# MathisWellmann/gym-rs

Measured on AMD Instinct MI355X. Metric: env-steps/sec (whole node), CartPole-v1 @ 2^20 envs per MI355X, higher is better.
Workload: dtype f32

## Files before the change

### gym-rs_amd/csrc/gymrs_engine.hip

```cpp
#include "gymrs_engine_priv.h"

static thread_local std::string g_last_error;

gymrs_status fail(gymrs_status st, const std::string& msg)
{
    g_last_error = msg;
    return st;
}


constexpr int kMaxDevices = 64;
static std::atomic<const gymrs_engine*> g_last_stepper[kMaxDevices];
static std::atomic<uint32_t> g_stepper_run[kMaxDevices];
constexpr uint32_t kTakeOverAfter = 64;

static size_t action_size(gymrs_env_kind kind) { return kind == GYMRS_PENDULUM ? sizeof(float) : sizeof(uint8_t); }

constexpr uint64_t kHostPoolMaxLanes = 64;

static uint64_t os_entropy()
{
    std::random_device rd;
    return ((uint64_t)rd() << 32) ^ (uint64_t)rd();
}
// ... 75 lines not shown
}

gymrs_status fold_reset_log(gymrs_engine* e)
{
    if (!e->reset_log || e->log_pending == 0) return GYMRS_OK;
    if (gymrs_status st = stream_op_barrier(e)) return st;
    HIP_TRY(launch_fold_reset_log(e->reset_log, e->log_row_words, e->log_first_tick, e->log_pending, e->log_vec, e->ep_start, e->n,
                                  e->block_stats, e->stream));
    e->log_pending = 0;
    return GYMRS_OK;
}

static bool launch_is_logged(const gymrs_engine* e, uint32_t flags)
{
    return e->reset_log && (flags & GYMRS_TRACK_STATS) && (flags & GYMRS_AUTO_RESET) && !(flags & GYMRS_TIME_LIMIT);
}

static gymrs_status log_before_step(gymrs_engine* e, uint32_t flags, uint32_t* fold)
{
    *fold = 0;
    if (!e->reset_log) return GYMRS_OK;
    const ResetLogStep s = reset_log_step({e->log_pending, e->log_first_tick, e->log_vec}, launch_is_logged(e, flags), e->tick, e->vec);
    if (s.fold_first)
        if (gymrs_status st = fold_reset_log(e)) return st;
    e->log_pending = s.after.pending;
    e->log_first_tick = s.after.first_tick;
    e->log_vec = s.after.vec;
    *fold = s.fold_step;
    return GYMRS_OK;
}
// ... 458 lines not shown
    }
    e->n_stat_blocks = (uint32_t)((((n_envs + 255) / 256) + 15) / 16 * 16);
    chk(dev_alloc(&e->block_stats, (size_t)e->n_stat_blocks * 2));
    constexpr uint32_t kAllThree = GYMRS_AUTO_RESET | GYMRS_TRACK_STATS | GYMRS_TIME_LIMIT;
    e->limit_elidable = kind == GYMRS_CARTPOLE && (flags & kAllThree) == kAllThree;
    {
        constexpr uint64_t kElideRewardFromBytes = 128ull << 20;
        bool on = kind == GYMRS_CARTPOLE && (flags & GYMRS_AUTO_RESET) && bytes_per_step(kind, e->state_dim, n_envs) >= kElideRewardFromBytes;
        if (const char* v = std::getenv("GYMRS_DEV_ELIDE_REWARD"))
            if (kind == GYMRS_CARTPOLE && (flags & GYMRS_AUTO_RESET) && (v[0] == '0' || v[0] == '1')) on = v[0] == '1';
        e->elide_reward = on;
    }
    if ((flags & GYMRS_TRACK_STATS) && (flags & GYMRS_AUTO_RESET) && kind == GYMRS_CARTPOLE &&
        (!(flags & GYMRS_TIME_LIMIT) || e->limit_elidable)) {
        e->log_row_words = e->n_stat_blocks * 4;
        chk(dev_alloc(&e->reset_log, (size_t)kResetLogRows * e->log_row_words));
    }
    if (e->limit_elidable) {
        chk(dev_alloc(&e->age_dev, (size_t)kStatsPartials));
        if (st == GYMRS_OK && mapped_host_block(2 * sizeof(uint32_t), &e->age_host, &e->age_host_dev) != hipSuccess)
            st = fail(GYMRS_EHIP, "hipHostMalloc (age words)");
    }
    chk(dev_alloc(&e->wave_open, (size_t)e->n_stat_blocks));
    chk(dev_alloc(&e->wave_clean, (size_t)e->n_stat_blocks));
    chk(dev_alloc(&e->err, 2));
    if (st == GYMRS_OK && mapped_host_block(2 * sizeof(uint32_t), &e->err_seen, &e->err_seen_dev) != hipSuccess)
        st = fail(GYMRS_EHIP, "hipHostMalloc (error flags)");
    chk(dev_alloc(&e->stats_dev, 4));
    if (st == GYMRS_OK && mapped_host_block(4 * sizeof(double), &e->stats_host, &e->stats_host_dev) != hipSuccess)
        st = fail(GYMRS_EHIP, "hipHostMalloc (statistics read-out)");
    chk(dev_alloc(&e->stats_acc, (size_t)kStatsPartials * 3));
    chk(dev_alloc(&e->stats_base, (size_t)kStatsBaseWords));
    chk(dev_alloc(&e->tick_dev, 1));
    if (st != GYMRS_OK) {
        std::string msg = g_last_error;
        gymrs_engine_destroy(e);
        return fail(st, msg);
    }
    hipError_t serr = hipStreamCreateWithFlags(&e->stream, hipStreamNonBlocking);
    if (serr != hipSuccess) {
        gymrs_engine_destroy(e);
        return fail(GYMRS_EHIP, std::string("hipStreamCreate: ") + hipGetErrorString(serr));
    }
    e->own_stream = true;
    static const uint32_t err_init[2] = {0u, 0xffffffffu};
    hipError_t merr = hipMemcpyAsync(e->err, err_init, sizeof(err_init), hipMemcpyHostToDevice, e->stream);
    if (merr == hipSuccess && e->reset_log) merr = hipMemsetAsync(e->reset_log, 0, (size_t)kResetLogRows * e->log_row_words * 8, e->stream);
    if (merr == hipSuccess) merr = hipMemsetAsync(e->truncated, 0, npad, e->stream);
    if (merr == hipSuccess) merr = hipMemsetAsync(e->stats_dev, 0, 4 * sizeof(double), e->stream);
    if (merr != hipSuccess) {
        gymrs_engine_destroy(e);
        return fail(GYMRS_EHIP, std::string("engine init: ") + hipGetErrorString(merr));
    }
    st = gymrs_reset(e, 0, 0, nullptr, nullptr);
    if (st == GYMRS_OK) st = gymrs_sync(e);
    if (st != GYMRS_OK) {
        std::string msg = g_last_error;
        gymrs_engine_destroy(e);
        return fail(st, msg);
    }
    if (aql_enabled_by_env() && !e->pool_host) {
        e->aql_tried = true;
// ... 23 lines not shown
gymrs_status gymrs_get_stream(gymrs_engine* e, void** hip_stream)
{
    if (!e || !hip_stream) return fail(GYMRS_EINVAL, "gymrs_get_stream: NULL argument");
    *hip_stream = e->stream;
    return GYMRS_OK;
}

gymrs_status gymrs_set_tuning(gymrs_engine* e, int lanes_per_thread, int memory_hint)
{
    if (!e) return fail(GYMRS_EINVAL, "gymrs_set_tuning: engine is NULL");
    if (lanes_per_thread != 4 && lanes_per_thread != 8)
        return fail(GYMRS_EINVAL, "gymrs_set_tuning: lanes_per_thread must be 4 or 8");
    if (memory_hint < 0 || memory_hint > 3) return fail(GYMRS_EINVAL, "gymrs_set_tuning: memory_hint must be 0, 1, 2 or 3");
    e->vec = lanes_per_thread;
    e->nt_mode = memory_hint;
    return GYMRS_OK;
}

static double default_reset_low_f64(gymrs_env_kind kind, int) { return kind == GYMRS_CARTPOLE ? -0.05 : -0.6; }
static double default_reset_high_f64(gymrs_env_kind kind, int) { return kind == GYMRS_CARTPOLE ? 0.05 : -0.4; }

struct PcgReset {
    const uint64_t* seeds_dev;
    double low[4], scale[4];
};

static gymrs_status reset_lanes(gymrs_engine* e, uint64_t seed, const float* lo, const float* hi, const PcgReset* pcg)
{
    std::memcpy(e->lo, lo, sizeof(e->lo));
    std::memcpy(e->hi, hi, sizeof(e->hi));
    if (gymrs_status st = fold_reset_log(e)) return st;
    e->seed = seed;
    e->tick = 0;
    if (e->graph_exec) {
        (void)hipGraphExecDestroy(e->graph_exec);
        e->graph_exec = nullptr;
    }

    ResetArgs a;
    std::memset(&a, 0, sizeof(a));
    for (int j = 0; j < 4; ++j) a.s[j] = e->s[j];
    a.obs_cos = e->obs_cos;
    a.obs_sin = e->obs_sin;
    a.reward = e->reward;
    a.done = e->done;
    a.truncated = e->truncated;
    a.beyond = e->beyond;
    a.ep_start = e->ep_start;
// ... 115 lines not shown
    e->open_vec = vec;
    return GYMRS_OK;
}

struct StepLaunch {
    uint32_t flags;
    StepArgs args;
};

static gymrs_status prepare_step(gymrs_engine* e, const void* actions, bool chain, StepLaunch* l)
{
    l->flags = take_over_device(e, launch_flags_of(e));
    if (gymrs_status st = elide_time_limit(e, &l->flags)) return st;
    if (chain) l->flags = (l->flags & ~kFlagHintMask) | hint_bits(e->nt_mode, bytes_per_step(e->kind, e->state_dim, e->n), true);
    l->args = step_args(e, actions);
    return log_before_step(e, l->flags, &l->args.fold_step);
}

static void record_step(gymrs_engine* e, const StepLaunch& l, int path)
{
    e->last_flags = l.flags;
    e->last_path = path;
    if (has_uniform_clock(e)) {
        e->trunc_held = (int)l.args.truncate_all;
        e->uniform_start = uniform_clock_after(e->tick, e->uniform_start, l.args.truncate_all != 0, (e->flags & GYMRS_AUTO_RESET) != 0);
    }
    e->tick += 1;
    if (path == 2) e->aql_launches += 1;
    e->n_steps_total += (double)e->n;
}

static hipError_t launch_step_through_hip_module(gymrs_engine* e, uint32_t flags, const StepArgs& a);

static gymrs_status step_through_hip(gymrs_engine* e, const void* actions)
{
    StepLaunch l;
    if (gymrs_status st = prepare_step(e, actions, false, &l)) return st;
    const uint32_t flags = l.flags;
    const StepArgs& a = l.args;
    if ((e->dev_hooks & 8u) && !(e->flags & GYMRS_FINAL_OBS) && !e->table_k)
        HIP_TRY(launch_step_through_hip_module(e, flags, a));
    else
// ... 34 lines not shown
    Policy,
    Exploring,
};
struct RolloutRequest {
    ActionSource actions;
    uint64_t action_seed = 0, action_t0 = 0;
    bool fitness = false;
    const gymrs_trajectory* record = nullptr;
    const TransitionArgs* transitions = nullptr;
};

static gymrs_status rollout_impl(gymrs_engine* e, uint32_t n_steps, const RolloutRequest& q)
{
    if (n_steps == 0) return GYMRS_OK;
    HIP_TRY(hipSetDevice(e->device));
    StepArgs a = step_args(e, nullptr);
    a.skip_trunc_store = 0;
    RolloutArgs r;
    std::memset(&r, 0, sizeof(r));
    r.action_seed = q.action_seed;
    r.action_t0 = q.action_t0;
    r.uniform_start = e->uniform_start;
    r.n_steps = n_steps;
    r.n_actions = e->kind == GYMRS_CARTPOLE ? 2u : 3u;
    r.max_torque = e->max_torque;
    int vec = e->vec == 8 ? 8 : 4;
    if (const gymrs_trajectory* rec = q.record) {
        r.rec_obs = rec->obs;
        r.rec_action = rec->actions;
        r.rec_reward = rec->reward;
// ... 147 lines not shown
    HIP_TRY(hipMemcpyAsync(e->action_staging, actions_host, bytes, hipMemcpyHostToDevice, e->stream));
    return gymrs_step(e, e->action_staging);
}

static gymrs_status build_graph(gymrs_engine* e, const char* base, uint64_t stride_bytes, uint32_t n_buffers, uint32_t steps)
{
    if (e->graph_exec) {
        (void)hipGraphExecDestroy(e->graph_exec);
        e->graph_exec = nullptr;
    }
    hipGraph_t graph = nullptr;
    HIP_TRY(hipStreamBeginCapture(e->stream, hipStreamCaptureModeThreadLocal));
    hipError_t err = hipSuccess;
    const uint32_t flags = launch_flags_of(e);
    ResetLogRing ring{0, 0, e->vec};
    for (uint32_t t = 0; t < steps && err == hipSuccess; ++t) {
        StepArgs a = step_args(e, base + (size_t)(t % n_buffers) * stride_bytes);
        a.tick = t;
        a.tick_base = e->tick_dev;
        const ResetLogStep s = reset_log_step(ring, launch_is_logged(e, flags), t, e->vec);
        a.fold_step = s.fold_step;
        ring = s.after;
        err = launch_step(e->kind, e->vec, flags, a, launch_consts(e), e->stream);
    }
    if (err == hipSuccess) err = launch_tick_advance(e->tick_dev, steps, e->stream);
    hipError_t end = hipStreamEndCapture(e->stream, &graph);
    if (err != hipSuccess || end != hipSuccess) {
        if (graph) (void)hipGraphDestroy(graph);
        return fail(GYMRS_EHIP, std::string("HIP graph capture: ") + hipGetErrorString(err != hipSuccess ? err : end));
    }
    err = hipGraphInstantiate(&e->graph_exec, graph, nullptr, nullptr, 0);
    (void)hipGraphDestroy(graph);
    if (err != hipSuccess) return fail(GYMRS_EHIP, std::string("hipGraphInstantiate: ") + hipGetErrorString(err));
    e->graph_actions = base;
    e->graph_stride = stride_bytes;
    e->graph_nbuf = n_buffers;
    e->graph_steps = steps;
// ... 163 lines not shown
        if (n_steps >= per_graph) {
            const bool hit = e->graph_exec && e->graph_actions == base && e->graph_stride == stride_bytes &&
                             e->graph_nbuf == n_buffers && e->graph_steps == per_graph && e->graph_flags == launch_flags_of(e) &&
                             e->graph_vec == e->vec && e->graph_seed == e->seed;
            if (!hit) {
                if (gymrs_status st = build_graph(e, base, stride_bytes, n_buffers, per_graph)) return st;
            }
            const unsigned long long tick_now = e->tick;
            HIP_TRY(hipMemcpyAsync(e->tick_dev, &tick_now, sizeof(tick_now), hipMemcpyHostToDevice, e->stream));
            HIP_TRY(hipStreamSynchronize(e->stream));
            if (gymrs_status st = fold_reset_log(e)) return st;
            if (e->device >= 0 && e->device < kMaxDevices) {
                g_last_stepper[e->device].store(e, std::memory_order_relaxed);
                g_stepper_run[e->device].store(kTakeOverAfter, std::memory_order_relaxed);
            }
            while (n_steps - done >= per_graph) {
                HIP_TRY(hipGraphLaunch(e->graph_exec, e->stream));
                done += per_graph;
                e->tick += per_graph;
                e->n_steps_total += (double)e->n * (double)per_graph;
            }
            if (e->flags & GYMRS_TIME_LIMIT) e->trunc_zero = false;
        }
    }
    if (!use_graph && aql_usable(e, n_steps - done)) {
        bool taken = false;
        if (gymrs_status st = step_many_aql(e, base, stride_bytes, n_buffers, done, n_steps, &taken)) return st;
        if (taken) done = n_steps;
    }
    for (uint32_t t = done; t < n_steps; ++t)
// ... 60 lines not shown
```

### gym-rs_amd/csrc/gymrs_engine_io.hip

```cpp
#include "gymrs_engine_priv.h"
#include "gymrs_evaluate.h"

static RcclApi g_rccl;

void comm_destroy(gymrs_engine* e)
{
    if (e->comm && g_rccl.CommDestroy) g_rccl.CommDestroy(e->comm);
    e->comm = nullptr;
}

extern "C" {

gymrs_status gymrs_obs_ptrs(gymrs_engine* e, float** out_ptrs, int* obs_dim)
{
    if (!e || !out_ptrs || !obs_dim) return fail(GYMRS_EINVAL, "gymrs_obs_ptrs: NULL argument");
    if (e->kind == GYMRS_PENDULUM) {
        out_ptrs[0] = e->obs_cos;
        out_ptrs[1] = e->obs_sin;
        out_ptrs[2] = e->s[1];
    } else {
        for (int j = 0; j < e->obs_dim; ++j) out_ptrs[j] = e->s[j];
    }
    *obs_dim = e->obs_dim;
    return GYMRS_OK;
// ... 90 lines not shown
        if (gymrs_status st_ = stream_sync_checked(e)) return st_;
        for (int j = 0; j < e->state_dim; ++j) std::memcpy(host_out + (size_t)j * count, host_of(e, e->s[j]) + first, count * sizeof(float));
        return GYMRS_OK;
    }
    for (int j = 0; j < e->state_dim; ++j)
        HIP_TRY(hipMemcpyAsync(host_out + (size_t)j * count, e->s[j] + first, count * sizeof(float), hipMemcpyDeviceToHost, e->stream));
    if (gymrs_status st_ = stream_sync_checked(e)) return st_;
    return GYMRS_OK;
}

gymrs_status gymrs_set_state(gymrs_engine* e, uint64_t first, uint64_t count, const float* host_in)
{
    if (!e || !host_in) return fail(GYMRS_EINVAL, "gymrs_set_state: NULL argument");
    if (gymrs_status st = range_check(e, first, count, "gymrs_set_state")) return st;
    HIP_TRY(hipSetDevice(e->device));
    if (e->pool_host) {
        HIP_TRY(hipStreamSynchronize(e->stream));
        for (int j = 0; j < e->state_dim; ++j) std::memcpy(host_of(e, e->s[j]) + first, host_in + (size_t)j * count, count * sizeof(float));
        if (e->kind == GYMRS_PENDULUM)
            for (uint64_t i = 0; i < count; ++i) sincosf_(host_in[i], host_of(e, e->obs_sin) + first + i, host_of(e, e->obs_cos) + first + i);
        return GYMRS_OK;
    }
    for (int j = 0; j < e->state_dim; ++j)
        HIP_TRY(hipMemcpyAsync(e->s[j] + first, host_in + (size_t)j * count, count * sizeof(float), hipMemcpyHostToDevice, e->stream));
    if (e->kind == GYMRS_PENDULUM) {
        std::vector<float> c(count), s(count);
        for (uint64_t i = 0; i < count; ++i) sincosf_(host_in[i], &s[i], &c[i]);
        HIP_TRY(hipMemcpyAsync(e->obs_cos + first, c.data(), count * sizeof(float), hipMemcpyHostToDevice, e->stream));
        HIP_TRY(hipMemcpyAsync(e->obs_sin + first, s.data(), count * sizeof(float), hipMemcpyHostToDevice, e->stream));
        HIP_TRY(hipStreamSynchronize(e->stream));
// ... 88 lines not shown
    dst->max_steps = src->max_steps;
    std::memcpy(dst->lo, src->lo, sizeof(dst->lo));
    std::memcpy(dst->hi, src->hi, sizeof(dst->hi));
    std::memcpy(dst->dflt_lo, src->dflt_lo, sizeof(dst->dflt_lo));
    std::memcpy(dst->dflt_hi, src->dflt_hi, sizeof(dst->dflt_hi));
    dst->epoch = src->epoch;
    dst->seed = src->seed;
    dst->tick = src->tick;
    dst->uniform_start = src->uniform_start;
    dst->n_steps_total = src->n_steps_total;
    dst->vec = src->vec;
    dst->nt_mode = src->nt_mode;
    dst->open_vec = src->open_vec;
    dst->trunc_held = src->trunc_held;
    limit_restart(dst, src->start_bound, src->trunc_zero);
    *dst->err_seen = 1u;
}
}
}

gymrs_status gymrs_engine_clone(gymrs_engine* src, gymrs_engine** out)
{
    if (!src || !out) return fail(GYMRS_EINVAL, "gymrs_engine_clone: NULL argument");
    *out = nullptr;
    gymrs_engine* dst = nullptr;
    if (gymrs_status st = gymrs_engine_create(src->kind, src->n, src->gid0, src->device, nullptr, src->flags, &dst)) return st;
    copy_scalars(dst, src);
    if (gymrs_status st = fold_reset_log(src)) {
        gymrs_engine_destroy(dst);
        return st;
// ... 117 lines not shown
    if (table_k) {
        p += sizeof(table_k);
        if (gymrs_status st = gymrs_set_param_table(e, p, (uint32_t)table_k)) return st;
        p += (size_t)table_k * params_size(e->kind);
        HIP_TRY(hipMemcpyAsync(e->param_index, p, (size_t)e->n * sizeof(uint16_t), hipMemcpyHostToDevice, e->stream));
    } else {
        if (e->table_k) drop_graph(e);
        e->table_k = 0;
    }
    HIP_TRY(hipStreamSynchronize(e->stream));
    e->gid0 = h.gid0;
    e->epoch = h.epoch;
    e->max_steps = h.max_steps;
    e->seed = h.seed;
    e->tick = h.tick;
    e->uniform_start = h.uniform_start;
    e->n_steps_total = h.n_steps_total;
    std::memcpy(e->lo, h.lo, sizeof(e->lo));
    std::memcpy(e->hi, h.hi, sizeof(e->hi));
    e->max_torque = h.max_torque;
    e->open_vec = (int)h.open_vec;
    e->trunc_held = -1;
    limit_restart(e, 0, false);
    *e->err_seen = 1u;
    HIP_TRY(hipMemsetAsync(e->wave_clean, 0, (size_t)e->n_stat_blocks * sizeof(uint32_t), e->stream));
    e->clean_shape = 0;
    std::memcpy(&e->consts, h.consts, h.consts_bytes);
    std::memcpy(&e->params, h.params, sizeof(e->params));
    return GYMRS_OK;
}
// ... 455 lines not shown
                                        "time and keeps a lane's step count in 32 bits); split the evaluation");
    if (gymrs_status st = ensure_policy_eval(e, "gymrs_evaluate_policy")) return st;
    HIP_TRY(hipSetDevice(e->device));
    HIP_TRY(launch_policy_eval_identity(e->eval_dev, e->policy.n_policies, e->stream));
    EvalArgs a;
    std::memset(&a, 0, sizeof(a));
    a.n = e->n;
    a.gid0 = e->gid0;
    a.seed = d->seed;
    a.episodes = d->episodes_per_lane;
    a.max_steps = m;
    a.flags = d->flags & GYMRS_EVAL_COMMON_STARTS;
    a.lengths = d->lengths_dev;
    a.table = e->eval_dev;
    a.box = make_sample_box(e->dflt_lo, e->dflt_hi, e->state_dim);
    HIP_TRY(launch_evaluate_policy(e->kind, e->table_k ? kFlagTable : 0u, a, launch_consts(e), e->policy, e->stream));
    return GYMRS_OK;
}

gymrs_status gymrs_policy_eval_ptr(gymrs_engine* e, gymrs_policy_eval** dev_out, uint32_t* n_policies)
{
    if (!e || !dev_out) return fail(GYMRS_EINVAL, "gymrs_policy_eval_ptr: NULL argument");
    if (gymrs_status st = ensure_policy_eval(e, "gymrs_policy_eval_ptr")) return st;
    *dev_out = e->eval_dev;
    if (n_policies) *n_policies = e->policy.n_policies;
    return GYMRS_OK;
}

gymrs_status gymrs_get_policy_eval(gymrs_engine* e, uint32_t first, uint32_t count, gymrs_policy_eval* host_out)
{
// ... 14 lines not shown
        e->params.cp = *static_cast<const gymrs_cartpole_params*>(params);
        e->consts.cp = make_consts(e->params.cp);
        break;
    case GYMRS_MOUNTAIN_CAR:
        e->params.mc = *static_cast<const gymrs_mountain_car_params*>(params);
        e->consts.mc = make_consts(e->params.mc);
        break;
    case GYMRS_PENDULUM:
        e->params.pd = *static_cast<const gymrs_pendulum_params*>(params);
        e->consts.pd = make_consts(e->params.pd);
        e->max_steps = e->consts.pd.max_steps;
        e->max_torque = (float)e->params.pd.max_torque;
        break;
    }
    e->table_k = 0;
    drop_graph(e);
    return GYMRS_OK;
}

gymrs_status gymrs_get_params(gymrs_engine* e, void* params_out)
{
    if (!e || !params_out) return fail(GYMRS_EINVAL, "gymrs_get_params: NULL argument");
    switch (e->kind) {
    case GYMRS_CARTPOLE: *static_cast<gymrs_cartpole_params*>(params_out) = e->params.cp; break;
    case GYMRS_MOUNTAIN_CAR: *static_cast<gymrs_mountain_car_params*>(params_out) = e->params.mc; break;
    case GYMRS_PENDULUM: *static_cast<gymrs_pendulum_params*>(params_out) = e->params.pd; break;
    }
    return GYMRS_OK;
}

// ... 7 lines not shown
    if (gymrs_status st = stream_sync_checked(e)) return st;
    if (v >= e->table_k)
        return fail(GYMRS_EINVAL, std::string(who) + ": lane " + std::to_string(lane) + " has parameter index " + std::to_string(v) +
                                      ", which is not below the table's " + std::to_string(e->table_k) + " rows");
    *idx = v;
    return GYMRS_OK;
}
const void* table_row(const gymrs_engine* e, uint32_t idx) { return e->table_params.data() + (size_t)idx * params_size(e->kind); }
}
}

gymrs_status gymrs_set_param_table(gymrs_engine* e, const void* rows, uint32_t k)
{
    static const char* who = "gymrs_set_param_table";
    if (!e) return fail(GYMRS_EINVAL, "gymrs_set_param_table: NULL engine");
    if (e->kind == GYMRS_PENDULUM)
        return fail(GYMRS_EINVAL, "gymrs_set_param_table: Pendulum engines take no parameter table (its max_torque also drives the random-policy actions)");
    if (!rows && k == 0) {
        if (e->table_k) drop_graph(e);
        e->table_k = 0;
        return GYMRS_OK;
    }
    if (!rows) return fail(GYMRS_EINVAL, "gymrs_set_param_table: rows is NULL but k > 0");
    if (k == 0) return fail(GYMRS_EINVAL, "gymrs_set_param_table: k must be >= 1 (rows = NULL, k = 0 switches the table off)");
    if (k > kMaxParamRows) return fail(GYMRS_EINVAL, "gymrs_set_param_table: k must be <= 65536 (the lane index is 16 bits)");
    const size_t psz = params_size(e->kind);
    const unsigned char* rp = static_cast<const unsigned char*>(rows);
    std::vector<ParamRow> dev_rows(k);
    for (uint32_t i = 0; i < k; ++i) {
        const void* row = rp + (size_t)i * psz;
// ... 94 lines not shown
    if (gymrs_status st = lane_param_set(e, lane, &idx, "gymrs_get_lane_params")) return st;
    std::memcpy(params_out, table_row(e, idx), params_size(e->kind));
    return GYMRS_OK;
}

extern "C++" {
namespace {
json::Object engine_extras(const gymrs_engine* e, uint64_t lane, uint32_t max_episode_steps, uint32_t param_set)
{
    json::Object g;
    g.str("kind", e->kind == GYMRS_CARTPOLE ? "CartPole" : (e->kind == GYMRS_MOUNTAIN_CAR ? "MountainCar" : "Pendulum"));
    g.uint("n_envs", e->n).uint("global_env_id", e->gid0 + lane).uint("flags", e->flags).uint("seed", e->seed).uint("tick", e->tick);
    g.uint("max_episode_steps", max_episode_steps);
    if (e->table_k) g.uint("param_set", param_set).uint("param_table_rows", e->table_k);
    g.uint("aql_chains", e->aql_chains).uint("aql_launches", e->aql_launches);
    if (e->aql) g.str("aql_handover", e->aql_handover.c_str());
    if (e->last_path != 0) {
        const int threads = step_threads_of(e->kind, e->n, e->vec);
        const uint32_t h = e->last_flags & kFlagHintMask;
        const char* hint = (h & kFlagNonTemporal) ? "nt" : (h == (kFlagNtOut | kFlagNtStateLoads) ? "so" : (h == kFlagNtOut ? "o" : "pl"));
        char buf[160];
        if (e->last_path == 2)
            std::snprintf(buf, sizeof(buf), "chain: %s", aql_kernel_name(e, e->last_flags, threads).c_str());
        else
            std::snprintf(buf, sizeof(buf), "HIP launch: gymrs::step_kernel<%s%s%s, %d, flags %u | hint %s, %d work-items>",
                          (e->last_flags & kFlagTable) ? "TableT<" : "",
                          e->kind == GYMRS_CARTPOLE ? "CartPoleT" : (e->kind == GYMRS_MOUNTAIN_CAR ? "MountainCarT" : "PendulumT"),
                          (e->last_flags & kFlagTable) ? ">" : "", e->vec, e->last_flags & 7u, hint, threads);
        g.str("last_launch", buf);
    }
// ... 16 lines not shown
    json::Object m;
    m.raw("render_modes", arr).uint("render_fps", fps).null("marker");
    return m;
}
}
}

gymrs_status gymrs_env_json(gymrs_engine* e, uint64_t lane, char* buf, uint64_t cap, uint64_t* needed)
{
    if (!e || (!buf && cap != 0)) return fail(GYMRS_EINVAL, "gymrs_env_json: NULL argument");
    if (lane >= e->n) return fail(GYMRS_EINVAL, "gymrs_env_json: lane out of range");
    HIP_TRY(hipSetDevice(e->device));
    float st[4] = {0, 0, 0, 0};
    uint8_t beyond = 0;
    if (e->pool_host) {
        if (gymrs_status st_ = stream_sync_checked(e)) return st_;
        for (int j = 0; j < e->state_dim; ++j) st[j] = host_of(e, e->s[j])[lane];
        if (e->kind == GYMRS_CARTPOLE) beyond = host_of(e, e->beyond)[lane];
    } else {
        for (int j = 0; j < e->state_dim; ++j) HIP_TRY(hipMemcpyAsync(&st[j], e->s[j] + lane, sizeof(float), hipMemcpyDeviceToHost, e->stream));
        if (e->kind == GYMRS_CARTPOLE) HIP_TRY(hipMemcpyAsync(&beyond, e->beyond + lane, 1, hipMemcpyDeviceToHost, e->stream));
        if (gymrs_status st_ = stream_sync_checked(e)) return st_;
    }
    uint32_t set = 0;
    if (e->table_k)
        if (gymrs_status st_ = lane_param_set(e, lane, &set, "gymrs_env_json")) return st_;
    double low[4], high[4];
    int dim = 0;
    json::Object o;
    switch (e->kind) {
    case GYMRS_CARTPOLE: {
        const gymrs_cartpole_params& p = e->table_k ? *static_cast<const gymrs_cartpole_params*>(table_row(e, set)) : e->params.cp;
        gymrs_observation_space(e->kind, &p, low, high, &dim);
        static const char* names[4] = {"x", "x_dot", "theta", "theta_dot"};
        json::Object lo, hi, state;
        for (int j = 0; j < 4; ++j) {
// ... 194 lines not shown
```

### gym-rs_amd/csrc/gymrs_engine_priv.h

```cpp
#pragma once
#include <hip/hip_runtime.h>

#include <dlfcn.h>

#include <atomic>
#include <chrono>
#include <cmath>
#include <cstdio>
#include <cstdlib>
#include <cstring>
#include <limits>
#include <new>
#include <random>
#include <string>
#include <vector>

#include "gymrs_amd.h"
#include "gymrs_aql.h"
#include "gymrs_json.h"
#include "gymrs_kernels.h"
#include "gymrs_step_plan.h"

using namespace gymrs;

// ... 52 lines not shown
    uint8_t* beyond = nullptr;
    uint32_t* ep_start = nullptr;
    float* final_obs = nullptr;
    uint32_t* wave_clean = nullptr;
    int clean_shape = 0;
    bool elide_reward = false;
    double* wave_open = nullptr;
    int open_vec = 0;
    int trunc_held = -1;
    unsigned long long* block_stats = nullptr;
    uint32_t n_stat_blocks = 0;
    unsigned long long* reset_log = nullptr;
    uint32_t log_row_words = 0, log_pending = 0;
    uint64_t log_first_tick = 0;
    int log_vec = 4;
    void* pool = nullptr;
    size_t pool_bytes = 0;
    char* pool_host = nullptr;
    char* staging_host = nullptr;
    int vec = 4;
    int nt_mode = 0;
    unsigned long long* trace = nullptr;
    uint32_t* err = nullptr;
    volatile uint32_t* err_seen = nullptr;
    uint32_t* err_seen_dev = nullptr;
    double* stats_dev = nullptr;
    volatile double* stats_host = nullptr;
    double* stats_host_dev = nullptr;
    unsigned long long* stats_acc = nullptr;
    unsigned long long* stats_base = nullptr;
// ... 117 lines not shown
```

### gym-rs_amd/csrc/gymrs_kernels.h

```cpp
#pragma once
#include <hip/hip_runtime.h>

#include <cstddef>

#include "gymrs_launch.h"
#include "gymrs_physics.h"

namespace gymrs {

#ifdef GYMRS_EXP_BLOCK
constexpr int kBlock = GYMRS_EXP_BLOCK;
#else
constexpr int kBlock = 256;
#endif

struct alignas(16) ParamRow {
    float v[8];
};
constexpr uint32_t kMaxParamRows = 65536;
static_assert(offsetof(CartPoleConsts, integrator) == 8 * sizeof(float) && offsetof(MountainCarConsts, max_steps) == 7 * sizeof(float),
              "a ParamRow holds the leading floats of the env's Consts");
__host__ __device__ inline ParamRow param_row(const CartPoleConsts& c)
{
    return ParamRow{{c.gravity, c.tau, c.force_over_tm, c.pml_over_tm, c.len_43, c.len_mp_over_tm, c.theta_thr, c.x_thr}};
// ... 43 lines not shown
    float* reward;
    uint8_t* done;
    uint8_t* truncated;
    union {
        uint8_t* beyond;
        float* final_obs;
    };
    uint32_t* ep_start;
    uint32_t* wave_clean;
    double* wave_open;
    unsigned long long* block_stats;
    unsigned long long* reset_log;
    uint32_t reset_log_row_words;
    uint32_t fold_step;
    uint32_t elide_reward;
    uint32_t* err;
    uint32_t* err_seen;
    uint64_t n;
    uint64_t n_fast;
    uint64_t gid0;
    uint64_t seed;
    uint64_t tick;
    const unsigned long long* tick_base;
    SampleBox box;
    uint32_t truncate_all;
    uint32_t skip_trunc_store;
    unsigned long long* trace;
    uint32_t* xcc_table;
    uint32_t xcc_check;
    uint32_t xcc_seq;
    uint32_t trace_wpb;
};

static_assert(offsetof(StepArgs, final_obs) == offsetof(StepArgs, beyond) && sizeof(float*) == sizeof(uint8_t*) && sizeof(StepArgs) == 296,
              "GYMRS_FINAL_OBS shares the slot of `beyond`: the layout of StepArgs must not move");
__host__ __device__ inline uint64_t final_obs_stride(uint64_t n) { return (n + 15) & ~15ull; }

template <class Consts>
struct StepKernArgs {
    float* s0;
    float* s1;
    float* s2;
    float* s3;
    const void* action;
    uint64_t n_fast;
    StepArgs rest;
    Consts c;
};
static_assert(offsetof(StepKernArgs<TableConsts>, rest) == 6 * 8 && alignof(TableConsts) <= 8 && sizeof(StepArgs) % alignof(TableConsts) == 0 &&
                  offsetof(StepKernArgs<TableConsts>, c) == 6 * 8 + sizeof(StepArgs),
// ... 135 lines not shown
```

### gym-rs_amd/csrc/gymrs_physics.h

```cpp
#pragma once
#include "gymrs_amd.h"
#include "gymrs_math.h"
#include "gymrs_philox.h"

namespace gymrs {

GYMRS_HD float clipf(float v, float l, float r)
{
    if (!(v <= r)) return r;
    if (!(v >= l)) return l;
    return v;
}


inline float f32_not_above(double t)
{
    float f = (float)t;
    if ((double)f > t) f = __builtin_nextafterf(f, -__builtin_inff());
    return f;
}
inline float f32_not_below(double t)
{
    float f = (float)t;
    if ((double)f < t) f = __builtin_nextafterf(f, __builtin_inff());
// ... 43 lines not shown
    const float xacc = fmaf_(-c.pml_over_tm, thetaacc * costheta, temp);
    if (INTEG == 0 || (INTEG < 0 && c.integrator == 0)) {
        x = fmaf_(c.tau, x_dot, x);
        x_dot = fmaf_(c.tau, xacc, x_dot);
        theta = fmaf_(c.tau, theta_dot, theta);
        theta_dot = fmaf_(c.tau, thetaacc, theta_dot);
    } else {
        x_dot = fmaf_(c.tau, xacc, x_dot);
        x = fmaf_(c.tau, x_dot, x);
        theta_dot = fmaf_(c.tau, thetaacc, theta_dot);
        theta = fmaf_(c.tau, theta_dot, theta);
    }
    return !(fabsf_(x) <= c.x_thr) || !(fabsf_(theta) <= c.theta_thr);
}

GYMRS_HD float cartpole_reward(bool done, bool& beyond)
{
    if (!done) return 1.0f;
    if (!beyond) {
        beyond = true;
        return 1.0f;
    }
    return 0.0f;
}

GYMRS_HD void cartpole_sample(const u32x4& r, const SampleBox& b, float& x, float& x_dot, float& theta, float& theta_dot)
{
    x = uniform_in_box(r.v[0], b, 0);
    x_dot = uniform_in_box(r.v[1], b, 1);
    theta = uniform_in_box(r.v[2], b, 2);
// ... 103 lines not shown
```

### gym-rs_amd/csrc/gymrs_step_plan.h

```cpp
#pragma once
#include "gymrs_launch.h"

namespace gymrs {

inline uint64_t bytes_per_step(gymrs_env_kind kind, int state_dim, uint64_t n)
{
    return n * ((uint64_t)state_dim * 8 + 10 + (kind == GYMRS_PENDULUM ? 8 : 0));
}

constexpr uint64_t kHintAllUpToBytes = 48ull << 20;
constexpr uint64_t kHintAllFromBytes = 1024ull << 20;

inline uint32_t hint_bits(int nt_mode, uint64_t per_step, bool chain)
{
    switch (nt_mode) {
    case 1: return kFlagNonTemporal;
    case 2: return 0u;
    case 3: return kFlagNtOut;
    default: break;
    }
    if (per_step >= kHintAllFromBytes) return kFlagNonTemporal;
    if (per_step > kHintAllUpToBytes) return kFlagNtOut;
    return chain ? (kFlagNtOut | kFlagNtStateLoads) : kFlagNonTemporal;
}
// ... 19 lines not shown
    }
    if (!logged) return s;
    if (s.after.pending == 0) {
        s.after.first_tick = tick;
        s.after.vec = vec;
    }
    if (s.after.pending == kResetLogRows - 1) {
        s.fold_step = 1;
        s.after.pending = 0;
    } else {
        s.after.pending += 1;
    }
    return s;
}

inline uint32_t graph_steps(uint32_t n_buffers, bool logged)
{
    uint32_t passes = (32 + n_buffers - 1) / n_buffers;
    if (logged) {
        uint32_t g = n_buffers, r = kResetLogRows;
        while (r) {
            const uint32_t tmp = g % r;
            g = r;
            r = tmp;
        }
        const uint32_t unit = kResetLogRows / g;
        passes = (passes + unit - 1) / unit * unit;
    }
    return n_buffers * passes;
}
// ... 9 lines not shown
```

### gym-rs_amd/csrc/gymrs_tile.h

```cpp
#pragma once
#include <type_traits>

#include "gymrs_kernels.h"

namespace gymrs {


#ifdef GYMRS_TRACE_TIMES
#define GYMRS_STAMP(slot_)                                                                                   \
    do {                                                                                                     \
        if (a.trace && (threadIdx.x & 63u) == 0)                                                             \
            a.trace[((size_t)blockIdx.x * a.trace_wpb + (threadIdx.x >> 6)) * 8 + (slot_)] = __builtin_amdgcn_s_memtime(); \
    } while (0)
#else
#define GYMRS_STAMP(slot_) do { } while (0)
#endif

__device__ __forceinline__ float wave_sum(float v)
{
    auto dpp_add = [](float x, auto ctrl, auto row_mask) {
        const int moved = __builtin_amdgcn_update_dpp(0, __builtin_bit_cast(int, x), decltype(ctrl)::value, decltype(row_mask)::value, 0xf, true);
        return x + __builtin_bit_cast(float, moved);
    };
    using std::integral_constant;
// ... 410 lines not shown
    } else {
#pragma unroll
        for (int k = 0; k < VEC; ++k) {
            if (need_reset[k]) {
#pragma unroll
                for (int j = 0; j < Env::kState; ++j) fo[(uint64_t)j * stride + base + k] = ls[j][k];
            }
        }
    }
}

struct NoFinalSink {
    static constexpr bool kOn = false;
};

template <class Env, int VEC, uint32_t FLAGS, bool FULL, bool ROLL = false, int THREADS = Env::kThreads, class Sink = NoFinalSink>
__device__ __forceinline__ void advance_tile(const StepArgs& a, const typename Env::Consts& c, uint64_t base,
                                             TileRegs<Env, VEC, FLAGS>& d, ResetLds<Env, VEC, THREADS>& lds, unsigned long long& resets,
                                             double& ret, double& open, StepOut<VEC>& out, uint32_t vblock, const Sink* sink = nullptr)
{
    static_assert(Env::kConstReward || Env::kNeverTerminates,
                  "return tracking assumes a constant reward (return = +-length) or one shared episode clock");
    constexpr int kVec = VEC;
    using R = TileRegs<Env, VEC, FLAGS>;
    constexpr bool AUTO = R::AUTO, STATS = R::STATS, TLIM = R::TLIM;
    constexpr bool LOGGED = R::LOGGED && !ROLL;
    constexpr int NS = Env::kState;
    using Action = typename Env::Action;
    const uint32_t tick_next = (uint32_t)(a.tick + 1);

    float ls[NS][kVec];
    Action la[kVec];
#pragma unroll
    for (int k = 0; k < kVec; ++k) {
        la[k] = d.act.v[k];
#pragma unroll
        for (int j = 0; j < NS; ++j) ls[j][k] = d.st[j].v[k];
    }
    float rw[kVec];
    bool dn[kVec], tr[kVec], need_reset[kVec];
#ifdef GYMRS_TRACE_TIMES
    asm volatile("s_waitcnt vmcnt(0)" ::: "memory");
    GYMRS_STAMP(2);
#endif
// ... 97 lines not shown
#ifdef GYMRS_EXP_EARLY_OUT
    if (!ROLL && !Env::kElideConstReward) {
#pragma unroll
        for (int k = 0; k < kVec; ++k) out.reward.v[k] = rw[k];
        store_vec<float, kVec, R::POL_O>(a.reward, base, a.n, FULL, out.reward);
        if (!Env::kNeverTerminates) store_vec<uint8_t, kVec, R::POL_O>(a.done, base, a.n, FULL, out.done);
        if (TLIM && !(Env::kNeverTerminates && a.skip_trunc_store)) store_vec<uint8_t, kVec, R::POL_O>(a.truncated, base, a.n, FULL, out.trunc);
    }
#endif
    if (AUTO) {
        constexpr int LPW = 64 * kVec;
        const uint32_t tid = threadIdx.x, wave = tid >> 6, lane = tid & 63u;
        uint16_t* list = lds.list + wave * LPW;
        uint32_t slot[kVec];
        uint32_t total = 0;
#pragma unroll
        for (int k = 0; k < kVec; ++k) {
            const unsigned long long m = __ballot(need_reset[k]);
            out.masks[k] = m;
            const uint32_t rank = __builtin_amdgcn_mbcnt_hi((uint32_t)(m >> 32), __builtin_amdgcn_mbcnt_lo((uint32_t)m, 0u));
            slot[k] = total + rank;
            if (need_reset[k]) {
                list[slot[k]] = (uint16_t)(lane * kVec + k);
            }
            total += (uint32_t)__popcll(m);
        }
        if (total != 0) {
            if constexpr (R::FINAL) store_final_obs<Env, VEC, FLAGS, FULL>(a, base, ls, need_reset);
            if constexpr (Sink::kOn) sink->store(base, ls, need_reset);
            if (LOGGED && a.fold_step == 0 && lane == 0) {
                typedef unsigned long long ull2 __attribute__((ext_vector_type(2)));
                const size_t wave_slot = (size_t)vblock * (THREADS / 64) + wave;
                ull2* row = reinterpret_cast<ull2*>(a.reset_log + (size_t)((uint32_t)a.tick & (kResetLogRows - 1u)) * a.reset_log_row_words +
                                                    wave_slot * kVec);
#pragma unroll
                for (int k = 0; k < kVec; k += 2) row[k / 2] = ull2{out.masks[k], out.masks[k + 1]};
            }
            __builtin_amdgcn_fence(__ATOMIC_RELEASE, "wavefront");
            __builtin_amdgcn_wave_barrier();
            const uint64_t wave_base = base - (uint64_t)lane * kVec;
            for (uint32_t i = lane; i < total; i += 64u) {
                const uint64_t gl = wave_base + list[i];
                const u32x4 r = draw4(a.seed, a.gid0 + gl, a.tick, kStreamReset);
                float ns[NS];
                Env::sample(r, a.box, ns);
                typename ResetLds<Env, VEC, THREADS>::State fs;
#pragma unroll
                for (int j = 0; j < NS; ++j) fs.v[j] = ns[j];
                lds.fresh[wave * LPW + i] = fs;
                if (!ROLL && !LOGGED && (STATS || TLIM)) a.ep_start[gl] = tick_next;
            }
            __builtin_amdgcn_fence(__ATOMIC_RELEASE, "wavefront");
            __builtin_amdgcn_wave_barrier();
#pragma unroll
            for (int k = 0; k < kVec; ++k) {
                if (need_reset[k]) {
                    const typename ResetLds<Env, VEC, THREADS>::State fs = lds.fresh[wave * LPW + slot[k]];
#pragma unroll
                    for (int j = 0; j < NS; ++j) ls[j][k] = fs.v[j];
                    if (ROLL && (STATS || TLIM)) d.ep_start.v[k] = tick_next;
                }
            }
            if (STATS && !LOGGED) {
                unsigned long long* bs = a.block_stats + ((size_t)vblock * (THREADS / 64) + wave) * 2;
                if (!Env::kConstReward) {
                    ret += open;
                    open = 0.0;
                    if (!ROLL && lane == 0) reinterpret_cast<double*>(bs)[1] = ret;
                }
                resets += total;
                if (!ROLL && lane == 0) bs[0] = resets;
            }
        }
    }
    GYMRS_STAMP(4);
#pragma unroll
    for (int k = 0; k < kVec; ++k) {
        out.reward.v[k] = rw[k];
#pragma unroll
        for (int j = 0; j < NS; ++j) d.st[j].v[k] = ls[j][k];
    }
}

template <class Env, int VEC, uint32_t FLAGS, bool FULL, bool ROLL = false>
__device__ __forceinline__ void store_tile(const StepArgs& a, uint64_t base, const TileRegs<Env, VEC, FLAGS>& d,
                                           const StepOut<VEC>& out, bool skip_reward = false)
// ... 40 lines not shown
```

Before: 151.7 billion.

## Predict next-step CartPole resets and pre-draw fresh states before stepping

After each step the kernel predicts which lanes will terminate on the next Euler step and writes those wave masks to a double-buffered hint row. On the next launch it reads the hint, builds the reset list and draws fresh reset states at the start of the tile, so the RNG and sampling work can overlap the physics. If the actual ballot masks match, the late list build and draw are skipped; otherwise it falls back and counts a miss atomically. In exchange every step pays an extra ballot pass, a hint-row write and a hint-row read, plus host bookkeeping to invalidate the hint on state-changing events.

```diff
diff --git a/gym-rs_amd/csrc/gymrs_engine.hip b/gym-rs_amd/csrc/gymrs_engine.hip
--- a/gym-rs_amd/csrc/gymrs_engine.hip
+++ b/gym-rs_amd/csrc/gymrs_engine.hip
@@ -113,6 +113,29 @@
 static bool launch_is_logged(const gymrs_engine* e, uint32_t flags)
 {
     return e->reset_log && (flags & GYMRS_TRACK_STATS) && (flags & GYMRS_AUTO_RESET) && !(flags & GYMRS_TIME_LIMIT);
+}
+
+static bool launch_writes_hint(const gymrs_engine* e, uint32_t flags)
+{
+    return rearm_hint_launch(e->kind, e->table_k != 0, e->vec, launch_is_logged(e, flags), flags);
+}
+static bool is_euler(const gymrs_engine* e) { return e->kind == GYMRS_CARTPOLE && e->consts.cp.integrator == 0; }
+
+static gymrs_status poison_hint_rows(gymrs_engine* e)
+{
+    if (gymrs_status st = stream_op_barrier(e)) return st;
+    unsigned long long* rows = e->reset_log + rearm_hint_row_at(e->log_row_words, 0);
+    const size_t bytes = (size_t)2 * e->log_row_words * 8;
+    if (e->dev_hooks & 256u) {
+        std::vector<unsigned long long> v((size_t)2 * e->log_row_words);
+        std::mt19937_64 rng(e->tick * 0x9e3779b97f4a7c15ull + 1u);
+        for (auto& w : v) w = rng();
+        HIP_TRY(hipMemcpyAsync(rows, v.data(), bytes, hipMemcpyHostToDevice, e->stream));
+        HIP_TRY(hipStreamSynchronize(e->stream));
+    } else {
+        HIP_TRY(hipMemsetAsync(rows, (e->dev_hooks & 64u) ? 0xff : 0x00, bytes, e->stream));
+    }
+    return GYMRS_OK;
 }
 
 static gymrs_status log_before_step(gymrs_engine* e, uint32_t flags, uint32_t* fold)
@@ -601,7 +624,7 @@
     if ((flags & GYMRS_TRACK_STATS) && (flags & GYMRS_AUTO_RESET) && kind == GYMRS_CARTPOLE &&
         (!(flags & GYMRS_TIME_LIMIT) || e->limit_elidable)) {
         e->log_row_words = e->n_stat_blocks * 4;
-        chk(dev_alloc(&e->reset_log, (size_t)kResetLogRows * e->log_row_words));
+        chk(dev_alloc(&e->reset_log, reset_log_alloc_words(e->log_row_words)));
     }
     if (e->limit_elidable) {
         chk(dev_alloc(&e->age_dev, (size_t)kStatsPartials));
@@ -632,7 +655,7 @@
     e->own_stream = true;
     static const uint32_t err_init[2] = {0u, 0xffffffffu};
     hipError_t merr = hipMemcpyAsync(e->err, err_init, sizeof(err_init), hipMemcpyHostToDevice, e->stream);
-    if (merr == hipSuccess && e->reset_log) merr = hipMemsetAsync(e->reset_log, 0, (size_t)kResetLogRows * e->log_row_words * 8, e->stream);
+    if (merr == hipSuccess && e->reset_log) merr = hipMemsetAsync(e->reset_log, 0, reset_log_alloc_words(e->log_row_words) * 8, e->stream);
     if (merr == hipSuccess) merr = hipMemsetAsync(e->truncated, 0, npad, e->stream);
     if (merr == hipSuccess) merr = hipMemsetAsync(e->stats_dev, 0, 4 * sizeof(double), e->stream);
     if (merr != hipSuccess) {
@@ -686,6 +709,7 @@
     if (memory_hint < 0 || memory_hint > 3) return fail(GYMRS_EINVAL, "gymrs_set_tuning: memory_hint must be 0, 1, 2 or 3");
     e->vec = lanes_per_thread;
     e->nt_mode = memory_hint;
+    e->hint = rearm_hint_after(HintEvent::ParamChange);
     return GYMRS_OK;
 }
 
@@ -704,6 +728,7 @@
     if (gymrs_status st = fold_reset_log(e)) return st;
     e->seed = seed;
     e->tick = 0;
+    e->hint = rearm_hint_after(HintEvent::Reset);
     if (e->graph_exec) {
         (void)hipGraphExecDestroy(e->graph_exec);
         e->graph_exec = nullptr;
@@ -849,7 +874,10 @@
     if (gymrs_status st = elide_time_limit(e, &l->flags)) return st;
     if (chain) l->flags = (l->flags & ~kFlagHintMask) | hint_bits(e->nt_mode, bytes_per_step(e->kind, e->state_dim, e->n), true);
     l->args = step_args(e, actions);
-    return log_before_step(e, l->flags, &l->args.fold_step);
+    if (gymrs_status st = log_before_step(e, l->flags, &l->args.fold_step)) return st;
+    l->args.hint_on = rearm_hint_on(e->hint, launch_writes_hint(e, l->flags), is_euler(e), e->vec, step_threads_of(e->kind, e->n, e->vec));
+    if (l->args.hint_on && (e->dev_hooks & (64u | 128u | 256u))) return poison_hint_rows(e);
+    return GYMRS_OK;
 }
 
 static void record_step(gymrs_engine* e, const StepLaunch& l, int path)
@@ -861,6 +889,8 @@
         e->uniform_start = uniform_clock_after(e->tick, e->uniform_start, l.args.truncate_all != 0, (e->flags & GYMRS_AUTO_RESET) != 0);
     }
     e->tick += 1;
+    e->hint_launches += l.args.hint_on;
+    e->hint = rearm_hint_after_step(launch_writes_hint(e, l.flags), is_euler(e), e->vec, step_threads_of(e->kind, e->n, e->vec));
     if (path == 2) e->aql_launches += 1;
     e->n_steps_total += (double)e->n;
 }
@@ -925,6 +955,7 @@
 {
     if (n_steps == 0) return GYMRS_OK;
     HIP_TRY(hipSetDevice(e->device));
+    e->hint = rearm_hint_after(HintEvent::FusedCall);
     StepArgs a = step_args(e, nullptr);
     a.skip_trunc_store = 0;
     RolloutArgs r;
@@ -1102,6 +1133,7 @@
     hipError_t err = hipSuccess;
     const uint32_t flags = launch_flags_of(e);
     ResetLogRing ring{0, 0, e->vec};
+    RearmHint baked = rearm_hint_after(HintEvent::GraphReplay);
     for (uint32_t t = 0; t < steps && err == hipSuccess; ++t) {
         StepArgs a = step_args(e, base + (size_t)(t % n_buffers) * stride_bytes);
         a.tick = t;
@@ -1109,6 +1141,9 @@
         const ResetLogStep s = reset_log_step(ring, launch_is_logged(e, flags), t, e->vec);
         a.fold_step = s.fold_step;
         ring = s.after;
+        a.hint_on = rearm_hint_on(baked, launch_writes_hint(e, flags), is_euler(e), e->vec, step_threads_of(e->kind, e->n, e->vec));
+        e->hint_launches += a.hint_on;
+        baked = rearm_hint_after_step(launch_writes_hint(e, flags), is_euler(e), e->vec, step_threads_of(e->kind, e->n, e->vec));
         err = launch_step(e->kind, e->vec, flags, a, launch_consts(e), e->stream);
     }
     if (err == hipSuccess) err = launch_tick_advance(e->tick_dev, steps, e->stream);
@@ -1302,6 +1337,7 @@
                 g_last_stepper[e->device].store(e, std::memory_order_relaxed);
                 g_stepper_run[e->device].store(kTakeOverAfter, std::memory_order_relaxed);
             }
+            e->hint = rearm_hint_after(HintEvent::GraphReplay);
             while (n_steps - done >= per_graph) {
                 HIP_TRY(hipGraphLaunch(e->graph_exec, e->stream));
                 done += per_graph;
diff --git a/gym-rs_amd/csrc/gymrs_engine_io.hip b/gym-rs_amd/csrc/gymrs_engine_io.hip
--- a/gym-rs_amd/csrc/gymrs_engine_io.hip
+++ b/gym-rs_amd/csrc/gymrs_engine_io.hip
@@ -128,6 +128,7 @@
     if (!e || !host_in) return fail(GYMRS_EINVAL, "gymrs_set_state: NULL argument");
     if (gymrs_status st = range_check(e, first, count, "gymrs_set_state")) return st;
     HIP_TRY(hipSetDevice(e->device));
+    e->hint = rearm_hint_after(HintEvent::SetState);
     if (e->pool_host) {
         HIP_TRY(hipStreamSynchronize(e->stream));
         for (int j = 0; j < e->state_dim; ++j) std::memcpy(host_of(e, e->s[j]) + first, host_in + (size_t)j * count, count * sizeof(float));
@@ -246,6 +247,7 @@
     dst->open_vec = src->open_vec;
     dst->trunc_held = src->trunc_held;
     limit_restart(dst, src->start_bound, src->trunc_zero);
+    dst->hint = rearm_hint_after(HintEvent::Clone);
     *dst->err_seen = 1u;
 }
 }
@@ -393,6 +395,7 @@
     e->max_steps = h.max_steps;
     e->seed = h.seed;
     e->tick = h.tick;
+    e->hint = rearm_hint_after(HintEvent::SnapshotLoad);
     e->uniform_start = h.uniform_start;
     e->n_steps_total = h.n_steps_total;
     std::memcpy(e->lo, h.lo, sizeof(e->lo));
@@ -878,6 +881,7 @@
     a.lengths = d->lengths_dev;
     a.table = e->eval_dev;
     a.box = make_sample_box(e->dflt_lo, e->dflt_hi, e->state_dim);
+    e->hint = rearm_hint_after(HintEvent::FusedCall);
     HIP_TRY(launch_evaluate_policy(e->kind, e->table_k ? kFlagTable : 0u, a, launch_consts(e), e->policy, e->stream));
     return GYMRS_OK;
 }
@@ -922,6 +926,7 @@
         break;
     }
     e->table_k = 0;
+    e->hint = rearm_hint_after(HintEvent::ParamChange);
     drop_graph(e);
     return GYMRS_OK;
 }
@@ -959,6 +964,7 @@
 {
     static const char* who = "gymrs_set_param_table";
     if (!e) return fail(GYMRS_EINVAL, "gymrs_set_param_table: NULL engine");
+    e->hint = rearm_hint_after(HintEvent::ParamChange);
     if (e->kind == GYMRS_PENDULUM)
         return fail(GYMRS_EINVAL, "gymrs_set_param_table: Pendulum engines take no parameter table (its max_torque also drives the random-policy actions)");
     if (!rows && k == 0) {
@@ -1083,6 +1089,7 @@
     g.uint("max_episode_steps", max_episode_steps);
     if (e->table_k) g.uint("param_set", param_set).uint("param_table_rows", e->table_k);
     g.uint("aql_chains", e->aql_chains).uint("aql_launches", e->aql_launches);
+    g.uint("rearm_hint_launches", e->hint_launches).uint("rearm_hint_misses", e->hint_misses);
     if (e->aql) g.str("aql_handover", e->aql_handover.c_str());
     if (e->last_path != 0) {
         const int threads = step_threads_of(e->kind, e->n, e->vec);
@@ -1129,12 +1136,16 @@
     float st[4] = {0, 0, 0, 0};
     uint8_t beyond = 0;
     if (e->pool_host) {
+        if (e->reset_log)
+            HIP_TRY(hipMemcpyAsync(&e->hint_misses, e->reset_log + rearm_hint_misses_at(e->log_row_words), sizeof(e->hint_misses), hipMemcpyDeviceToHost, e->stream));
         if (gymrs_status st_ = stream_sync_checked(e)) return st_;
         for (int j = 0; j < e->state_dim; ++j) st[j] = host_of(e, e->s[j])[lane];
         if (e->kind == GYMRS_CARTPOLE) beyond = host_of(e, e->beyond)[lane];
     } else {
         for (int j = 0; j < e->state_dim; ++j) HIP_TRY(hipMemcpyAsync(&st[j], e->s[j] + lane, sizeof(float), hipMemcpyDeviceToHost, e->stream));
         if (e->kind == GYMRS_CARTPOLE) HIP_TRY(hipMemcpyAsync(&beyond, e->beyond + lane, 1, hipMemcpyDeviceToHost, e->stream));
+        if (e->reset_log)
+            HIP_TRY(hipMemcpyAsync(&e->hint_misses, e->reset_log + rearm_hint_misses_at(e->log_row_words), sizeof(e->hint_misses), hipMemcpyDeviceToHost, e->stream));
         if (gymrs_status st_ = stream_sync_checked(e)) return st_;
     }
     uint32_t set = 0;
diff --git a/gym-rs_amd/csrc/gymrs_engine_priv.h b/gym-rs_amd/csrc/gymrs_engine_priv.h
--- a/gym-rs_amd/csrc/gymrs_engine_priv.h
+++ b/gym-rs_amd/csrc/gymrs_engine_priv.h
@@ -90,6 +90,9 @@
     uint32_t log_row_words = 0, log_pending = 0;
     uint64_t log_first_tick = 0;
     int log_vec = 4;
+    RearmHint hint;
+    unsigned long long hint_misses = 0;
+    uint64_t hint_launches = 0;
     void* pool = nullptr;
     size_t pool_bytes = 0;
     char* pool_host = nullptr;
diff --git a/gym-rs_amd/csrc/gymrs_kernels.h b/gym-rs_amd/csrc/gymrs_kernels.h
--- a/gym-rs_amd/csrc/gymrs_kernels.h
+++ b/gym-rs_amd/csrc/gymrs_kernels.h
@@ -81,6 +81,7 @@
     uint32_t reset_log_row_words;
     uint32_t fold_step;
     uint32_t elide_reward;
+    uint32_t hint_on;
     uint32_t* err;
     uint32_t* err_seen;
     uint64_t n;
@@ -101,6 +102,9 @@
 
 static_assert(offsetof(StepArgs, final_obs) == offsetof(StepArgs, beyond) && sizeof(float*) == sizeof(uint8_t*) && sizeof(StepArgs) == 296,
               "GYMRS_FINAL_OBS shares the slot of `beyond`: the layout of StepArgs must not move");
+__host__ __device__ inline size_t rearm_hint_row_at(uint32_t row_words, uint32_t parity) { return (size_t)(kResetLogRows + (parity & 1u)) * row_words; }
+__host__ __device__ inline size_t rearm_hint_misses_at(uint32_t row_words) { return (size_t)(kResetLogRows + 2u) * row_words; }
+__host__ __device__ inline size_t reset_log_alloc_words(uint32_t row_words) { return rearm_hint_misses_at(row_words) + 1; }
 __host__ __device__ inline uint64_t final_obs_stride(uint64_t n) { return (n + 15) & ~15ull; }
 
 template <class Consts>
diff --git a/gym-rs_amd/csrc/gymrs_physics.h b/gym-rs_amd/csrc/gymrs_physics.h
--- a/gym-rs_amd/csrc/gymrs_physics.h
+++ b/gym-rs_amd/csrc/gymrs_physics.h
@@ -81,6 +81,13 @@
     return !(fabsf_(x) <= c.x_thr) || !(fabsf_(theta) <= c.theta_thr);
 }
 
+GYMRS_HD bool cartpole_will_finish(const CartPoleConsts& c, float x, float x_dot, float theta, float theta_dot)
+{
+    x = fmaf_(c.tau, x_dot, x);
+    theta = fmaf_(c.tau, theta_dot, theta);
+    return !(fabsf_(x) <= c.x_thr) || !(fabsf_(theta) <= c.theta_thr);
+}
+
 GYMRS_HD float cartpole_reward(bool done, bool& beyond)
 {
     if (!done) return 1.0f;
diff --git a/gym-rs_amd/csrc/gymrs_step_plan.h b/gym-rs_amd/csrc/gymrs_step_plan.h
--- a/gym-rs_amd/csrc/gymrs_step_plan.h
+++ b/gym-rs_amd/csrc/gymrs_step_plan.h
@@ -57,6 +57,37 @@
     return s;
 }
 
+enum class HintEvent {
+    Reset,
+    SetState,
+    SnapshotLoad,
+    Clone,
+    ParamChange,
+    FusedCall,
+    GraphReplay,
+};
+
+struct RearmHint {
+    bool armed = false;
+    int vec = 0;
+    int threads = 0;
+};
+
+inline bool rearm_hint_launch(gymrs_env_kind kind, bool table, int vec, bool logged, uint32_t flags)
+{
+    return kind == GYMRS_CARTPOLE && !table && vec == 4 && logged && !(flags & GYMRS_FINAL_OBS);
+}
+
+inline uint32_t rearm_hint_on(const RearmHint& h, bool writes, bool euler, int vec, int threads)
+{
+    return (writes && euler && h.armed && h.vec == vec && h.threads == threads) ? 1u : 0u;
+}
+inline RearmHint rearm_hint_after_step(bool writes, bool euler, int vec, int threads)
+{
+    return RearmHint{writes && euler, vec, threads};
+}
+inline RearmHint rearm_hint_after(HintEvent) { return RearmHint{}; }
+
 inline uint32_t graph_steps(uint32_t n_buffers, bool logged)
 {
     uint32_t passes = (32 + n_buffers - 1) / n_buffers;
diff --git a/gym-rs_amd/csrc/gymrs_tile.h b/gym-rs_amd/csrc/gymrs_tile.h
--- a/gym-rs_amd/csrc/gymrs_tile.h
+++ b/gym-rs_amd/csrc/gymrs_tile.h
@@ -448,6 +448,46 @@
     static constexpr bool kOn = false;
 };
 
+#define GYMRS_REARM_LIST_APPEND(list_, lane_, k_, m_, mine_, slot_, total_)                                                                  \
+    do {                                                                                                                                    \
+        const uint32_t rank = __builtin_amdgcn_mbcnt_hi((uint32_t)((m_) >> 32), __builtin_amdgcn_mbcnt_lo((uint32_t)(m_), 0u));               \
+        slot_[k_] = total_ + rank;                                                                                                          \
+        if (mine_) {                                                                                                                        \
+            list_[slot_[k_]] = (uint16_t)((lane_) * kVec + (k_));                                                       \
+        }                                                                                                                                   \
+        total_ += (uint32_t)__popcll(m_);                                                                                                   \
+    } while (0)
+#define GYMRS_REARM_DRAW_LISTED(list_, wave_, lane_, total_)                                                                                 \
+    do {                                                                                                                                    \
+        __builtin_amdgcn_fence(__ATOMIC_RELEASE, "wavefront");                                                                              \
+        __builtin_amdgcn_wave_barrier();                                                                                                    \
+        const uint64_t wave_base = base - (uint64_t)(lane_) * kVec;                               \
+        for (uint32_t i = (lane_); i < (total_); i += 64u) {                                   \
+            const uint64_t gl = wave_base + list_[i];                                                                                       \
+            const u32x4 r = draw4(a.seed, a.gid0 + gl, a.tick, kStreamReset);                                                               \
+            float ns[NS];                                                                                                                   \
+            Env::sample(r, a.box, ns);                                                                                                      \
+            typename ResetLds<Env, VEC, THREADS>::State fs;                                                                                 \
+            _Pragma("unroll") for (int j = 0; j < NS; ++j) fs.v[j] = ns[j];                                                                 \
+            lds.fresh[(wave_) * LPW + i] = fs;                                                                                              \
+                           \
+            if (!ROLL && !LOGGED && (STATS || TLIM)) a.ep_start[gl] = tick_next;                                                            \
+        }                                                                                                                                   \
+        __builtin_amdgcn_fence(__ATOMIC_RELEASE, "wavefront");                                                                              \
+        __builtin_amdgcn_wave_barrier();                                                                                                    \
+    } while (0)
+
+template <class Env>
+constexpr bool kRearmHintEnv = std::is_same_v<Env, CartPoleT>;
+template <bool ON, int VEC>
+struct RearmHintRegs {};
+template <int VEC>
+struct RearmHintRegs<true, VEC> {
+    bool hint_used;
+    unsigned long long hinted[VEC];
+    uint32_t hinted_slot[VEC], hinted_total;
+};
+
 template <class Env, int VEC, uint32_t FLAGS, bool FULL, bool ROLL = false, int THREADS = Env::kThreads, class Sink = NoFinalSink>
 __device__ __forceinline__ void advance_tile(const StepArgs& a, const typename Env::Consts& c, uint64_t base,
                                              TileRegs<Env, VEC, FLAGS>& d, ResetLds<Env, VEC, THREADS>& lds, unsigned long long& resets,
@@ -462,6 +502,33 @@
     constexpr int NS = Env::kState;
     using Action = typename Env::Action;
     const uint32_t tick_next = (uint32_t)(a.tick + 1);
+
+    constexpr bool HINT = kRearmHintEnv<Env> && kVec == 4 && R::LOGGED && !R::FINAL && !ROLL && !Sink::kOn;
+    [[maybe_unused]] RearmHintRegs<HINT, kVec> hr;
+    if constexpr (HINT && FULL) {
+        if (a.hint_on != 0) {
+            constexpr int LPW = 64 * kVec;
+            const uint32_t wave = threadIdx.x >> 6, lane = threadIdx.x & 63u;
+            uint16_t* list = lds.list + wave * LPW;
+            typedef unsigned long long ull4 __attribute__((ext_vector_type(4)));
+            typedef const __attribute__((address_space(4))) ull4* const_row_ptr;
+            const size_t wave_slot = (size_t)vblock * (THREADS / 64) + (uint32_t)__builtin_amdgcn_readfirstlane((int)wave);
+            const ull4 row = *(const_row_ptr)(a.reset_log + rearm_hint_row_at(a.reset_log_row_words, (uint32_t)a.tick) + wave_slot * kVec);
+            hr.hint_used = true;
+            hr.hinted_total = 0;
+#pragma unroll
+            for (int k = 0; k < kVec; ++k) {
+                hr.hinted[k] = row[k];
+                GYMRS_REARM_LIST_APPEND(list, lane, k, hr.hinted[k], ((hr.hinted[k] >> lane) & 1ull) != 0, hr.hinted_slot, hr.hinted_total);
+            }
+            if (hr.hinted_total != 0) GYMRS_REARM_DRAW_LISTED(list, wave, lane, hr.hinted_total);
+        } else {
+            hr.hint_used = false;
+        }
+        GYMRS_STAMP(7);
+    } else if constexpr (HINT) {
+        hr.hint_used = false;
+    }
 
     float ls[NS][kVec];
     Action la[kVec];
@@ -589,16 +656,33 @@
         uint16_t* list = lds.list + wave * LPW;
         uint32_t slot[kVec];
         uint32_t total = 0;
-#pragma unroll
-        for (int k = 0; k < kVec; ++k) {
-            const unsigned long long m = __ballot(need_reset[k]);
-            out.masks[k] = m;
-            const uint32_t rank = __builtin_amdgcn_mbcnt_hi((uint32_t)(m >> 32), __builtin_amdgcn_mbcnt_lo((uint32_t)m, 0u));
-            slot[k] = total + rank;
-            if (need_reset[k]) {
-                list[slot[k]] = (uint16_t)(lane * kVec + k);
-            }
-            total += (uint32_t)__popcll(m);
+        [[maybe_unused]] bool drawn = false;
+        if constexpr (HINT) {
+#pragma unroll
+            for (int k = 0; k < kVec; ++k) out.masks[k] = __ballot(need_reset[k]);
+            if (hr.hint_used) {
+                drawn = true;
+#pragma unroll
+                for (int k = 0; k < kVec; ++k) drawn = drawn && out.masks[k] == hr.hinted[k];
+                if (drawn) {
+                    total = hr.hinted_total;
+#pragma unroll
+                    for (int k = 0; k < kVec; ++k) slot[k] = hr.hinted_slot[k];
+                } else if (lane == 0) {
+                    atomicAdd(a.reset_log + rearm_hint_misses_at(a.reset_log_row_words), 1ull);
+                }
+            }
+            if (!drawn) {
+#pragma unroll
+                for (int k = 0; k < kVec; ++k) GYMRS_REARM_LIST_APPEND(list, lane, k, out.masks[k], need_reset[k], slot, total);
+            }
+        } else {
+#pragma unroll
+            for (int k = 0; k < kVec; ++k) {
+                const unsigned long long m = __ballot(need_reset[k]);
+                out.masks[k] = m;
+                GYMRS_REARM_LIST_APPEND(list, lane, k, m, need_reset[k], slot, total);
+            }
         }
         if (total != 0) {
             if constexpr (R::FINAL) store_final_obs<Env, VEC, FLAGS, FULL>(a, base, ls, need_reset);
@@ -611,22 +695,11 @@
 #pragma unroll
                 for (int k = 0; k < kVec; k += 2) row[k / 2] = ull2{out.masks[k], out.masks[k + 1]};
             }
-            __builtin_amdgcn_fence(__ATOMIC_RELEASE, "wavefront");
-            __builtin_amdgcn_wave_barrier();
-            const uint64_t wave_base = base - (uint64_t)lane * kVec;
-            for (uint32_t i = lane; i < total; i += 64u) {
-                const uint64_t gl = wave_base + list[i];
-                const u32x4 r = draw4(a.seed, a.gid0 + gl, a.tick, kStreamReset);
-                float ns[NS];
-                Env::sample(r, a.box, ns);
-                typename ResetLds<Env, VEC, THREADS>::State fs;
-#pragma unroll
-                for (int j = 0; j < NS; ++j) fs.v[j] = ns[j];
-                lds.fresh[wave * LPW + i] = fs;
-                if (!ROLL && !LOGGED && (STATS || TLIM)) a.ep_start[gl] = tick_next;
-            }
-            __builtin_amdgcn_fence(__ATOMIC_RELEASE, "wavefront");
-            __builtin_amdgcn_wave_barrier();
+            if constexpr (HINT) {
+                if (!drawn) GYMRS_REARM_DRAW_LISTED(list, wave, lane, total);
+            } else {
+                GYMRS_REARM_DRAW_LISTED(list, wave, lane, total);
+            }
 #pragma unroll
             for (int k = 0; k < kVec; ++k) {
                 if (need_reset[k]) {
@@ -645,6 +718,19 @@
                 }
                 resets += total;
                 if (!ROLL && lane == 0) bs[0] = resets;
+            }
+        }
+        if constexpr (HINT) {
+            if (Env::variant(c) == 0) {
+                unsigned long long next[kVec];
+#pragma unroll
+                for (int k = 0; k < kVec; ++k) next[k] = __ballot(cartpole_will_finish(c, ls[0][k], ls[1][k], ls[2][k], ls[3][k]));
+                if (lane == 0) {
+                    typedef unsigned long long ull2 __attribute__((ext_vector_type(2)));
+                    ull2* row = reinterpret_cast<ull2*>(a.reset_log + rearm_hint_row_at(a.reset_log_row_words, tick_next) + ((size_t)vblock * (THREADS / 64) + wave) * kVec);
+#pragma unroll
+                    for (int k = 0; k < kVec; k += 2) row[k / 2] = ull2{next[k], next[k + 1]};
+                }
             }
         }
     }
```

Result: slower. 149.4 billion (-1.5%).
